# sdroh1027/DiffusionVID

Measured on AMD Instinct MI355X. Metric: frames/sec (1000x600) DiffusionVID-R101 x1, higher is better.
Workload: dtype f16

## Files before the change

diffusionvid_amd/_lib.py:

```python
import ctypes as C
import os

_HERE = os.path.dirname(os.path.abspath(__file__))
LIB_PATH = os.environ.get("DVID_LIB") or os.path.join(_HERE, "libdvid_hip.so")

c_void_p, c_int, c_float, c_int64 = C.c_void_p, C.c_int, C.c_float, C.c_int64
c_float_p = C.POINTER(C.c_float)


class DvidConfig(C.Structure):
    _fields_ = [
        ("hidden_dim", c_int), ("nheads", c_int), ("dim_feedforward", c_int), ("dim_dynamic", c_int),
        ("num_classes", c_int), ("num_cls", c_int), ("num_reg", c_int), ("num_heads", c_int),
        ("num_heads_cond", c_int), ("pooler_resolution", c_int), ("sampling_ratio", c_int),
        ("res_blocks", c_int * 4), ("pixel_mean", c_float * 3), ("pixel_std", c_float * 3),
        ("backbone_type", c_int), ("swin_embed_dim", c_int), ("swin_depths", c_int * 4), ("swin_heads", c_int * 4),
        ("swin_window", c_int),
    ]


SIGNATURES = {
    "dvid_last_error": (C.c_char_p, []),
    "dvid_version": (c_int, []),
    "dvid_model_create": (c_int, [C.POINTER(DvidConfig), C.POINTER(c_void_p)]),
    "dvid_model_destroy": (c_int, [c_void_p]),
    "dvid_model_set_tensor": (c_int, [c_void_p, C.c_char_p, c_void_p, C.POINTER(c_int64), c_int]),
    "dvid_model_finalize": (c_int, [c_void_p]),
    "dvid_model_set_precision": (c_int, [c_void_p, c_int]),
    "dvid_model_take_range_flag": (c_int, [c_void_p, C.POINTER(c_int), c_void_p]),
    "dvid_set_chains": (c_int, [c_void_p, c_int]),
    "dvid_set_stem_layout": (c_int, [c_void_p, c_int]),
    "dvid_workspace_reserve": (c_int, [c_void_p, c_int, c_int, c_int, c_int]),
    "dvid_workspace_generation": (C.c_ulonglong, [c_void_p]),
    "dvid_backbone_resnet_fpn": (c_int, [c_void_p, c_void_p, c_int, c_int, c_int, c_void_p, c_void_p, c_void_p, c_void_p]),
    "dvid_backbone_swin_fpn": (c_int, [c_void_p, c_void_p, c_int, c_int, c_int, c_void_p, c_void_p, c_void_p, c_void_p]),
    "dvid_backbone_resnet_fpn_frames": (c_int, [c_void_p, c_void_p, c_int, c_int, c_int, c_void_p, c_void_p, c_void_p, c_void_p]),
    "dvid_backbone_swin_fpn_frames": (c_int, [c_void_p, c_void_p, c_int, c_int, c_int, c_void_p, c_void_p, c_void_p, c_void_p]),
    "dvid_rcnn_head": (c_int, [c_void_p, c_int, c_int, c_void_p, c_void_p, c_void_p, c_int, c_int, c_int, c_int, c_void_p,
                               c_void_p, C.POINTER(c_int64), c_void_p, c_void_p, c_void_p, c_void_p, c_void_p, c_void_p]),
    "dvid_global_xattn": (c_int, [c_void_p, c_void_p, c_int, c_void_p, c_int, c_void_p, c_void_p]),
    "dvid_global_memory_project": (c_int, [c_void_p, c_void_p, c_int, c_void_p]),
    "dvid_local_memory_project": (c_int, [c_void_p, c_int, c_void_p, c_int, c_int, c_void_p]),
    "dvid_local_xattn": (c_int, [c_void_p, c_int, c_void_p, c_int, c_int, c_int, c_void_p, c_void_p]),
    "dvid_roialign_v2_multilevel": (c_int, [c_void_p, c_void_p, c_void_p, c_int, c_int, c_int, c_int, c_void_p, c_int,
                                            c_void_p, c_void_p, c_void_p]),
    "dvid_roialign_v2_multilevel_f32": (c_int, [c_void_p, c_void_p, c_void_p, c_int, c_int, c_int, c_int, c_void_p, c_int,
                                                c_void_p, c_void_p, c_void_p]),
    "dvid_conv2d_nhwc_f32": (c_int, [c_void_p] * 8 + [c_int] * 12 + [c_void_p]),
    "dvid_mha_f32": (c_int, [c_void_p] * 4 + [c_int] * 7 + [c_int64] * 3 + [c_void_p]),
    "dvid_swin_window_attn_f32": (c_int, [c_void_p] * 4 + [c_int] * 6 + [c_void_p]),
    "dvid_swin_window_attn_f32_ws": (c_int, [c_void_p] * 4 + [c_int] * 7 + [c_void_p]),
    "dvid_dynconv_f32": (c_int, [c_void_p] * 7 + [c_int, c_void_p]),
    "dvid_select_topk_features": (c_int, [c_void_p, c_int, c_int, c_int, c_int, c_int, c_void_p, c_int, c_void_p, c_void_p,
                                          c_void_p]),
    "dvid_counter_normal": (c_int, [c_void_p, C.c_int64, c_int, C.c_uint64, c_void_p]),
    "dvid_noise_to_boxes": (c_int, [c_void_p, c_void_p, c_int, c_float, c_float, c_float, c_void_p]),
    "dvid_ddim_renew_step": (c_int, [c_void_p] * 6 + [c_int] * 3 + [c_float] * 9 + [c_void_p]),
    "dvid_postproc_topk_nms": (c_int, [c_void_p, c_void_p, c_int, c_int, c_int, c_int, c_float, c_float, c_float, c_int,
                                       c_void_p, c_void_p, c_void_p, c_void_p, c_void_p, c_void_p]),
    "dvid_postproc_scratch_bytes": (c_int64, [c_int, c_int, c_int]),
    "dvid_topk_candidates_stream": (c_int, [c_void_p, c_void_p, c_int, c_int, c_int, c_int, c_void_p, c_void_p, c_void_p, c_void_p]),
    "dvid_nms_frames_tiled": (c_int, [c_void_p] * 3 + [c_int, c_int, c_float, c_float, c_float, c_int, c_int] + [c_void_p] * 6),
    "dvid_nms_tiled_scratch_bytes": (c_int64, [c_int, c_int]),
    "dvid_seq_nms_video": (c_int, [c_void_p] * 4 + [c_int] * 3 + [c_void_p] * 4 + [c_int64, c_void_p]),
    "dvid_seq_nms_scratch_bytes": (c_int64, [c_void_p, c_void_p, c_int, c_int]),
    "dvid_cdist": (c_int, [c_void_p, c_int, c_int, c_void_p, c_void_p]),
    "dvid_fps_greedy": (c_int, [c_void_p, c_int, c_int, c_int, c_void_p, c_void_p]),
    "dvid_gather_rows": (c_int, [c_void_p, c_void_p, c_void_p, c_int, c_int, c_void_p]),
    "dvid_conv2d_nhwc_f16": (c_int, [c_void_p, c_void_p, c_void_p, c_void_p, c_void_p] + [c_int] * 13 + [c_void_p]),
    "dvid_bottleneck64_tail_f16": (c_int, [c_void_p] * 10 + [c_int] + [c_void_p] * 2 + [c_int] * 3 + [c_void_p]),
    "dvid_bottleneck128_tail_f16": (c_int, [c_void_p] * 10 + [c_int] * 3 + [c_void_p]),
    "dvid_mha_f16": (c_int, [c_void_p] * 5 + [c_int] * 7 + [c_int64] * 3 + [c_void_p]),
    "dvid_dynconv": (c_int, [c_void_p] * 7 + [c_int, c_void_p]),
    "dvid_add_layernorm": (c_int, [c_void_p] * 5 + [c_int, c_int, c_int, c_void_p]),
    "dvid_swin_pack_relbias": (c_int, [c_void_p, c_int, c_void_p]),
    "dvid_swin_window_attn_f16": (c_int, [c_void_p] * 4 + [c_int] * 6 + [c_void_p]),
    "dvid_swin_pack_relbias_ws": (c_int, [c_void_p, c_int, c_int, c_void_p]),
    "dvid_swin_window_attn_f16_ws": (c_int, [c_void_p] * 4 + [c_int] * 7 + [c_void_p]),
    "dvid_patch_merge_ln": (c_int, [c_void_p] * 5 + [c_int] * 4 + [c_void_p]),
    "dvid_nhwc_from_nchw": (c_int, [c_void_p, c_void_p, c_int, c_int, c_int, c_int, c_void_p]),
    "dvid_nchw_from_nhwc": (c_int, [c_void_p, c_void_p, c_int, c_int, c_int, c_int, c_void_p]),
    "dvid_f32_to_f16": (c_int, [c_void_p, c_void_p, c_int64, c_void_p]),
    "dvid_resize_u8_to_f32": (c_int, [c_void_p, c_int, c_int, c_void_p, c_void_p, c_int, c_int, c_int, c_int, c_void_p, c_void_p, c_int,
                                      c_void_p, c_void_p, c_int, c_void_p]),
    "dvid_igemm_num_configs": (c_int, []),
    "dvid_igemm_set_config": (c_int, [c_int]),
    "dvid_igemm_set_tuning": (c_int, [c_int]),
    "dvid_igemm_tuning_passes": (C.c_longlong, []),
    "dvid_igemm_set_conv3x3": (c_int, [c_int]),
    "dvid_igemm_set_wstat": (c_int, [c_int]),
    "dvid_igemm_set_bottleneck_fusion": (c_int, [c_int]),
    "dvid_set_stem_pool": (c_int, [c_int]),
    "dvid_set_option": (c_int, [C.c_char_p, c_int]),
    "dvid_get_option": (c_int, [C.c_char_p, C.POINTER(c_int)]),
    "dvid_reset_options": (c_int, []),
    "dvid_effective_config": (c_int, [C.c_char_p, c_int]),
    "dvid_profile_enable": (c_int, [c_int]),
    "dvid_profile_reset": (c_int, []),
# ... 54 lines not shown
```

diffusionvid_amd/csrc/dynconv.hip:

```cpp
#include "common.h"
#include "f32_split.h"
#include "igemm_epilogue.h"
#include "kernels.h"
#include "options.h"
#include "roi_taps.h"

namespace {

constexpr int NP = 49;
constexpr int D = 256;
constexpr int DD = 64;
constexpr int A_PITCH = D + 8;
constexpr int H_PITCH = DD + 8;

__device__ __forceinline__ float groups4_sum(float v) {
    v += __shfl_xor(v, 16, 64);
    v += __shfl_xor(v, 32, 64);
    return v;
}

template <bool FUSED_ROI>
__global__ __launch_bounds__(256, 3) void dynconv_kernel(const half_t* __restrict__ roi, const half_t* __restrict__ params,
                                                       const float* __restrict__ g1, const float* __restrict__ b1,
                                                       const float* __restrict__ g2, const float* __restrict__ b2,
                                                       half_t* __restrict__ out, RoiLevels lv, const float* __restrict__ boxes,
                                                       int boxes_per_img, int nbox) {
    extern __shared__ __attribute__((aligned(16))) char smem[];
    half_t* As = reinterpret_cast<half_t*>(smem);
    half_t* Hs = As + 64 * A_PITCH;
    float* red = reinterpret_cast<float*>(Hs + 64 * H_PITCH);

    const int box = FUSED_ROI ? igemm_xcd_remap((int)blockIdx.x, nbox) : (int)blockIdx.x;
    const int tid = threadIdx.x, lane = tid & 63, wave = tid >> 6;
    const int l15 = lane & 15, l4 = lane >> 4;
    const half_t* p1t = params + (long)box * (2 * D * DD);
    const half_t* p2t = p1t + D * DD;
    const half8 zero8 = {0, 0, 0, 0, 0, 0, 0, 0};
    half8 bf[8];
    half8 b2f[4][2];

    if (FUSED_ROI) {
#pragma unroll
        for (int ks = 0; ks < 8; ++ks)
            bf[ks] = *reinterpret_cast<const half8*>(p1t + (wave * 16 + l15) * D + ks * 32 + l4 * 8);
#pragma unroll
        for (int nt = 0; nt < 4; ++nt)
#pragma unroll
            for (int ks = 0; ks < 2; ++ks)
                b2f[nt][ks] = *reinterpret_cast<const half8*>(p2t + (wave * 64 + nt * 16 + l15) * DD + ks * 32 + l4 * 8);
        float macc[8];
        roi_taps::gather_box(lv, boxes, boxes_per_img, box, tid >> 5, tid & 31, macc,
                             [&](int p, half8 o) { *reinterpret_cast<half8*>(As + p * A_PITCH + (tid & 31) * 8) = o; });
        for (int i = tid; i < (64 - NP) * 32; i += 256) *reinterpret_cast<half8*>(As + (NP + (i >> 5)) * A_PITCH + (i & 31) * 8) = zero8;
    } else {
        const half_t* roi_b = roi + (long)box * NP * D;
        for (int i = tid; i < 64 * 32; i += 256) {
            const int r = i >> 5, cv = i & 31;
            const half8 v = *reinterpret_cast<const half8*>(roi_b + (long)(r < NP ? r : 0) * D + cv * 8);
            *reinterpret_cast<half8*>(As + r * A_PITCH + cv * 8) = (r < NP) ? v : zero8;
        }
#pragma unroll
        for (int ks = 0; ks < 8; ++ks)
            bf[ks] = *reinterpret_cast<const half8*>(p1t + (wave * 16 + l15) * D + ks * 32 + l4 * 8);
    }
    __syncthreads();

    float4v acc1[4];
#pragma unroll
    for (int mt = 0; mt < 4; ++mt) acc1[mt] = (float4v){0.f, 0.f, 0.f, 0.f};
#pragma unroll
    for (int ks = 0; ks < 8; ++ks) {
#pragma unroll
        for (int mt = 0; mt < 4; ++mt) {
            const half8 af = *reinterpret_cast<const half8*>(As + (mt * 16 + l15) * A_PITCH + ks * 32 + l4 * 8);
            acc1[mt] = __builtin_amdgcn_mfma_f32_16x16x32_f16(bf[ks], af, acc1[mt], 0, 0, 0);
        }
    }
    if (!FUSED_ROI) {
#pragma unroll
        for (int nt = 0; nt < 4; ++nt)
#pragma unroll
            for (int ks = 0; ks < 2; ++ks)
                b2f[nt][ks] = *reinterpret_cast<const half8*>(p2t + (wave * 64 + nt * 16 + l15) * DD + ks * 32 + l4 * 8);
    }

    float mean[4], rstd[4];
#pragma unroll
    for (int mt = 0; mt < 4; ++mt) {
        const float s = groups4_sum((acc1[mt][0] + acc1[mt][1]) + (acc1[mt][2] + acc1[mt][3]));
        if (l4 == 0) red[(mt * 16 + l15) * 4 + wave] = s;
    }
    __syncthreads();
#pragma unroll
    for (int mt = 0; mt < 4; ++mt) {
        const float4v t = *reinterpret_cast<const float4v*>(red + (mt * 16 + l15) * 4);
        mean[mt] = (t[0] + t[1] + t[2] + t[3]) * (1.f / DD);
    }
    __syncthreads();
#pragma unroll
    for (int mt = 0; mt < 4; ++mt) {
        float s = 0.f;
#pragma unroll
        for (int r = 0; r < 4; ++r) {
            const float c = acc1[mt][r] - mean[mt];
// ... 418 lines not shown
```

diffusionvid_amd/csrc/kernels.h:

```cpp
#pragma once
#include "common.h"

struct IgemmParams {
    const half_t* in;
    const half_t* w;
    const float* bias;
    const void* res;
    void* out;
    int H, W, Cin, Ho, Wo, Cout, KH, KW, stride, pad;
    int M, Kpad, ntaps, ldc, alg_k;
    int relu, out_f32, res_mode, res_f32;
    int splitk;
    long split_stride;
    int tiles_m, tiles_n;
};
int dvid_igemm_launch(const IgemmParams& p, hipStream_t s);
int dvid_igemm2_launch(const IgemmParams& p, hipStream_t s);

bool dvid_conv3x3_halo_supported(const IgemmParams& p);
bool dvid_conv3x3_halo_preferred(const IgemmParams& p);
int dvid_conv3x3_halo_launch(const IgemmParams& p, hipStream_t s);
bool dvid_stem_pool_supported(const IgemmParams& p);
int dvid_stem_pool_launch(const IgemmParams& p, hipStream_t s);

bool dvid_wstat_supported(const IgemmParams& p);
bool dvid_wstat_preferred(const IgemmParams& p);
int dvid_wstat_launch(const IgemmParams& p, hipStream_t s);

bool dvid_bneck64_tail_preferred(int H, int W);
int dvid_bneck128_tail_launch(const half_t* t1, const half_t* w2, const float* b2, const half_t* w3, const float* b3, const half_t* res,
                              const half_t* w1n, const float* b1n, half_t* out, half_t* t1n, int n, int H, int W, hipStream_t s);
int dvid_bneck64_tail_launch(const half_t* t1, const half_t* w2, const float* b2, const half_t* w3, const float* b3, const half_t* res,
                             const half_t* ws, const float* bs, const half_t* w1n, const float* b1n, int n_next, half_t* out, half_t* t1n,
                             int n, int H, int W, hipStream_t s);

struct FrameTable {
    static constexpr int kMax = 32;
    const float* p[kMax];
};
int dvid_prep_images_launch(const float* const* frames, half_t* nhwc8, int n, int h, int w, const float* mean, const float* inv_std,
                            hipStream_t s);
int dvid_prep_images_s2d_launch(const float* const* frames, half_t* s2d16, int n, int h, int w, const float* mean, const float* inv_std,
                                hipStream_t s);
int dvid_maxpool3x3s2_launch(const half_t* in, half_t* out, int n, int h, int w, int c, hipStream_t s);
int dvid_nchw_from_nhwc_launch(const half_t* in, float* out, int n, int h, int w, int c, hipStream_t s);
int dvid_nhwc_from_nchw_launch(const float* in, half_t* out, int n, int h, int w, int c, hipStream_t s);
int dvid_add_layernorm_launch(const float* x, const float* r, const float* g, const float* b, float* y32, half_t* y16,
                              int rows, int d, int relu, hipStream_t s, int nsplit = 1, long split_stride = 0,
                              const float* xbias = nullptr);
int dvid_f32_to_f16_launch(const float* x, half_t* y, long n, hipStream_t s);
int dvid_resize_u8_launch(const unsigned char* src, int h, int w, unsigned char* tmp, float* out, int oh, int ow, int ph, int pw,
                          const int* xbounds, const int* xk, int xksize, const int* ybounds, const int* yk, int yksize, hipStream_t s);
int dvid_modulate_launch(const float* x, const float* scale, int scale_ld, const float* shift, int shift_per_row, int shift_ld,
                         half_t* y16, int rows, int rows_per_frame, int d, hipStream_t s);
int dvid_silu_f16_launch(const float* x, half_t* y, long n, hipStream_t s);

template <typename T>
struct RoiLevelsT {
    const T* feat[3];
    int h[3], w[3];
    float scale[3];
};
using RoiLevels = RoiLevelsT<half_t>;
using RoiLevels32 = RoiLevelsT<float>;
int dvid_roialign_launch(const RoiLevels& lv, int channels, const float* boxes, int n_img, int boxes_per_img, half_t* roi_out,
                         float* mean_out, hipStream_t s);

int dvid_mha_mfma_launch(const half_t* q, const half_t* k, const half_t* v, half_t* out, half_t* vt_scratch, int batch, int lq,
                         int lk, int nheads, int q_ld, int kv_ld, int out_ld, long q_bs, long kv_bs, long out_bs, hipStream_t s);

struct OutProjLnParams {
    const void* x;
    int mode;
    const half_t* wf_hi;
    const half_t* wf_lo;
    const float* w32;
    const float* wscale;
    const float* bias;
    const float* gamma;
    const float* beta;
    float* out;
    int rows, d;
    int* range_flag;
};
int dvid_outproj_ln_launch(const OutProjLnParams& p, hipStream_t s);

constexpr int SWIN_RELBIAS_PITCH = 64;
int dvid_swin_window_attn_launch(const half_t* qkv, const half_t* qkv_bias16, const float* relbias, half_t* out, int batch, int H,
                                 int W, int C, int nheads, int shift, hipStream_t s);
constexpr int SWIN12_RELBIAS_PITCH = 160;
int dvid_swin_window12_attn_launch(const half_t* qkv, const half_t* qkv_bias16, const float* relbias, half_t* out, int batch, int H,
                                   int W, int C, int nheads, int shift, hipStream_t s);
int dvid_patch_merge_ln_launch(const float* x, const float* g, const float* b, half_t* y16, int B, int H, int W, int C, hipStream_t s,
                               float* y32 = nullptr);

int dvid_dynconv_launch(const half_t* roi, const half_t* params, const float* g1, const float* b1, const float* g2,
                        const float* b2, half_t* out, int rows, hipStream_t s);
int dvid_dynconv_roi_launch(const RoiLevels& lv, int channels, const float* boxes, int n_img, int boxes_per_img, const half_t* params,
                            const float* g1, const float* b1, const float* g2, const float* b2, half_t* out, hipStream_t s);

struct HeadTailParams {
    const half_t* x16;
    const float* obj32;
    const half_t* w1f;
    const float* b1;
    const half_t* w2f;
    const float* b2;
    const float* n3g;
    const float* n3b;
    const float* scale;
    int ss_stride, rows_per_frame;
    const float* cond32;
    const half_t* wcf;
    const float* bc;
    int num_cls, num_reg, num_classes, dff;
    const half_t* clsf[4];
    const float* clsg[4];
    const float* clsb[4];
    const half_t* regf[4];
// ... 87 lines not shown
```

diffusionvid_amd/csrc/ops_abi.hip:

```cpp
#include "runtime.h"

extern "C" {
int dvid_roialign_v2_multilevel(const void* p3, const void* p4, const void* p5, int n_frames, int height, int width, int channels,
                                const float* boxes, int boxes_per_frame, void* roi_out, float* mean_out, void* stream) {
    g_err[0] = 0;
    if (height % 32 || width % 32) FAIL(DVID_ERR_ARG, "height/width must be multiples of 32");
    TRY(dvid_roialign_launch(roi_levels<half_t>(p3, p4, p5, height, width, 0, channels), channels, boxes, n_frames, boxes_per_frame, reinterpret_cast<half_t*>(roi_out), mean_out,
                             reinterpret_cast<hipStream_t>(stream)));
    return DVID_OK;
}

int dvid_roialign_v2_multilevel_f32(const float* p3, const float* p4, const float* p5, int n_frames, int height, int width, int channels,
                                    const float* boxes, int boxes_per_frame, float* roi_out, float* mean_out, void* stream) {
    g_err[0] = 0;
    if (height % 32 || width % 32) FAIL(DVID_ERR_ARG, "height/width must be multiples of 32");
    TRY(dvid_f32_roialign_launch(roi_levels<float>(p3, p4, p5, height, width, 0, channels), channels, boxes, n_frames, boxes_per_frame, roi_out, mean_out, reinterpret_cast<hipStream_t>(stream)));
    return DVID_OK;
}

int dvid_conv2d_nhwc_f32(const float* in, const float* w, const void* w_hi, const void* w_lo, const float* bias, const float* row_scale, const float* residual,
                         float* out, int n, int h, int wd, int cin, int cout, int kh, int kw, int stride, int pad, int kpad, int relu, int residual_mode,
                         void* stream) {
    g_err[0] = 0;
    if (cin % 4 || kpad % 16 || kpad < kh * kw * cin || pad < 0) FAIL(DVID_ERR_ARG, "fp32 conv: cin %% 4 == 0, kpad %% 16 == 0, kpad >= kh*kw*cin, pad >= 0");
    ConvW cw;
    cw.w32 = const_cast<float*>(w);
    cw.w16hi = reinterpret_cast<half_t*>(const_cast<void*>(w_hi));
    cw.w16lo = reinterpret_cast<half_t*>(const_cast<void*>(w_lo));
    cw.bias = const_cast<float*>(bias);
    cw.wscale32 = const_cast<float*>(row_scale);
    cw.cin32 = cin;
    cw.cin_real = cin;
    cw.cout = cout;
    cw.kh = kh;
    cw.kw = kw;
    cw.stride = stride;
    cw.pad = pad;
    cw.kpad32 = kpad;
    TRY(conv_run32(cw, in, n, h, wd, out, reinterpret_cast<hipStream_t>(stream), {.relu = relu, .res = residual, .res_mode = residual_mode}));
    return DVID_OK;
}

int dvid_mha_f32(const float* q, const float* k, const float* v, float* out, int batch, int lq, int lk, int nheads, int q_ld, int kv_ld, int out_ld,
                 int64_t q_bs, int64_t kv_bs, int64_t out_bs, void* stream) {
    g_err[0] = 0;
    TRY(dvid_f32_mha_launch(q, k, v, out, batch, lq, lk, nheads, q_ld, kv_ld, out_ld, (long)q_bs, (long)kv_bs, (long)out_bs,
                            reinterpret_cast<hipStream_t>(stream)));
    return DVID_OK;
}

int dvid_swin_window_attn_f32(const float* qkv, const float* qkv_bias, const float* relbias, float* out, int batch, int H, int W, int C,
                              int nheads, int shift, void* stream) {
    g_err[0] = 0;
    if (!qkv || !qkv_bias || !relbias || !out) FAIL(DVID_ERR_ARG, "swin window attention: null pointer");
    if (batch <= 0 || H <= 0 || W <= 0 || nheads <= 0 || shift < 0 || shift >= 7)
        FAIL(DVID_ERR_ARG, "swin window attention: bad sizes (batch %d, %d x %d tokens, %d heads, shift %d)", batch, H, W, nheads, shift);
    const int rc = dvid_f32_swin_window_attn_launch(qkv, qkv_bias, relbias, out, batch, H, W, C, nheads, shift, reinterpret_cast<hipStream_t>(stream));
    if (rc != DVID_OK) FAIL(rc, "swin window attention (fp32): C %d with %d heads on %d x %d x %d tokens is not supported", C, nheads, batch, H, W);
    return DVID_OK;
}

// ... 291 lines not shown
```

diffusionvid_amd/csrc/roi_taps.h:

```cpp
#pragma once

#include "common.h"
#include "kernels.h"

namespace roi_taps {

constexpr int P = 7;
constexpr int G = 2;
constexpr int CV = 32;

typedef unsigned int uint4v __attribute__((ext_vector_type(4)));
__device__ __forceinline__ float mix_fma_lo(unsigned int h2, float w, float acc) {
    float d;
    asm("v_fma_mix_f32 %0, %1, %2, %3 op_sel_hi:[1,0,0]" : "=v"(d) : "v"(h2), "v"(w), "v"(acc));
    return d;
}
__device__ __forceinline__ float mix_fma_hi(unsigned int h2, float w, float acc) {
    float d;
    asm("v_fma_mix_f32 %0, %1, %2, %3 op_sel:[1,0,0] op_sel_hi:[1,0,0]" : "=v"(d) : "v"(h2), "v"(w), "v"(acc));
    return d;
}
__device__ __forceinline__ void tap_fma8(float (&acc)[8], half8 v, float w) {
    const uint4v u = __builtin_bit_cast(uint4v, v);
#pragma unroll
    for (int q = 0; q < 4; ++q) {
        acc[2 * q] = mix_fma_lo(u[q], w, acc[2 * q]);
        acc[2 * q + 1] = mix_fma_hi(u[q], w, acc[2 * q + 1]);
    }
}

struct Tap {
    int lo, hi;
    float wl, wh;
    bool ok;
};

__device__ __forceinline__ Tap axis_tap(float y, int limit) {
    Tap t;
    t.ok = !(y < -1.0f || y > (float)limit);
    if (y <= 0.f) y = 0.f;
    int lo = (int)y;
    int hi;
    if (lo >= limit - 1) {
        hi = lo = limit - 1;
        y = (float)lo;
    } else {
        hi = lo + 1;
    }
    const float l = y - (float)lo;
    t.lo = lo;
    t.hi = hi;
    t.wl = 1.f - l;
    t.wh = l;
    return t;
}

__device__ __forceinline__ int box_level(float bx1, float by1, float bx2, float by2, bool& valid) {
    const float area = (bx2 - bx1) * (by2 - by1);
    valid = area >= 0.f;
    float lvf = floorf(4.f + log2f(sqrtf(area) / 224.f + 1e-8f));
    lvf = fminf(fmaxf(lvf, 3.f), 5.f);
    return valid ? (int)lvf - 3 : 0;
}

template <typename Sink>
__device__ __forceinline__ void gather_box(const RoiLevels& lv, const float* __restrict__ boxes, int boxes_per_img, int box, int grp, int ln,
                                           float (&macc)[8], Sink&& sink) {
    const int img = box / boxes_per_img;
    const float bx1 = boxes[box * 4 + 0], by1 = boxes[box * 4 + 1], bx2 = boxes[box * 4 + 2], by2 = boxes[box * 4 + 3];
    bool valid_box;
    const int level = box_level(bx1, by1, bx2, by2, valid_box);

    const half_t* feat = lv.feat[level];
    const int H = lv.h[level], W = lv.w[level];
    const float sc = lv.scale[level];
    feat += (long)img * H * W * (CV * 8);

    const float x1 = bx1 * sc - 0.5f, y1 = by1 * sc - 0.5f;
    const float x2 = bx2 * sc - 0.5f, y2 = by2 * sc - 0.5f;
    const float bin_w = (x2 - x1) / P, bin_h = (y2 - y1) / P;

#pragma unroll
    for (int e = 0; e < 8; ++e) macc[e] = 0.f;

    for (int p = grp; p < P * P; p += 8) {
        const int ph = p / P, pw = p - ph * P;
        float acc[8];
#pragma unroll
        for (int e = 0; e < 8; ++e) acc[e] = 0.f;
        if (valid_box) {
#pragma unroll
            for (int iy = 0; iy < G; ++iy) {
                const float y = y1 + ph * bin_h + (iy + 0.5f) * bin_h / G;
                const Tap ty = axis_tap(y, H);
#pragma unroll
                for (int ix = 0; ix < G; ++ix) {
                    const float x = x1 + pw * bin_w + (ix + 0.5f) * bin_w / G;
                    const Tap tx = axis_tap(x, W);
                    if (!(ty.ok && tx.ok)) continue;
                    const half8 v1 = *reinterpret_cast<const half8*>(feat + ((long)ty.lo * W + tx.lo) * (CV * 8) + ln * 8);
                    const half8 v2 = *reinterpret_cast<const half8*>(feat + ((long)ty.lo * W + tx.hi) * (CV * 8) + ln * 8);
                    const half8 v3 = *reinterpret_cast<const half8*>(feat + ((long)ty.hi * W + tx.lo) * (CV * 8) + ln * 8);
                    const half8 v4 = *reinterpret_cast<const half8*>(feat + ((long)ty.hi * W + tx.hi) * (CV * 8) + ln * 8);
                    const float w1 = ty.wl * tx.wl, w2 = ty.wl * tx.wh, w3 = ty.wh * tx.wl, w4 = ty.wh * tx.wh;
                    tap_fma8(acc, v1, w1);
                    tap_fma8(acc, v2, w2);
                    tap_fma8(acc, v3, w3);
                    tap_fma8(acc, v4, w4);
                }
            }
        }
        half8 o;
#pragma unroll
        for (int e = 0; e < 8; ++e) {
            acc[e] *= 1.f / (G * G);
            macc[e] += acc[e];
            o[e] = (half_t)acc[e];
        }
        sink(p, o);
    }
}

}
```

diffusionvid_amd/csrc/roialign.hip:

```cpp
#include <stdlib.h>

#include "common.h"
#include "igemm_epilogue.h"
#include "kernels.h"
#include "roi_taps.h"

namespace {

using namespace roi_taps;

__global__ __launch_bounds__(256) void roialign_kernel(RoiLevels lv, const float* __restrict__ boxes, int boxes_per_img,
                                                        half_t* __restrict__ roi_out, float* __restrict__ mean_out, int nbox,
                                                        int xcd_major) {
    __shared__ float red[8][256];
    const int box = xcd_major ? igemm_xcd_remap((int)blockIdx.x, nbox) : (int)blockIdx.x;
    const int tid = threadIdx.x;
    const int grp = tid >> 5, ln = tid & 31;
    float macc[8];
    gather_box(lv, boxes, boxes_per_img, box, grp, ln, macc,
               [&](int p, half8 o) { *reinterpret_cast<half8*>(roi_out + ((long)box * (P * P) + p) * (CV * 8) + ln * 8) = o; });
    if (mean_out) {
#pragma unroll
        for (int e = 0; e < 8; ++e) red[grp][ln * 8 + e] = macc[e];
        __syncthreads();
        float s = 0.f;
#pragma unroll
        for (int g = 0; g < 8; ++g) s += red[g][tid];
        mean_out[(long)box * 256 + tid] = s / (P * P);
    }
}

__global__ __launch_bounds__(256) void f32_roialign_kernel(RoiLevels32 lv, const float* __restrict__ boxes, int boxes_per_img,
                                                            float* __restrict__ roi_out, float* __restrict__ mean_out, int nbox) {
#pragma clang fp contract(off)
    __shared__ float red[8][256];
    const int box = igemm_xcd_remap((int)blockIdx.x, nbox);
    const int img = box / boxes_per_img;
    const int tid = threadIdx.x;
    const int grp = tid >> 5, ln = tid & 31;
    const float bx1 = boxes[box * 4 + 0], by1 = boxes[box * 4 + 1], bx2 = boxes[box * 4 + 2], by2 = boxes[box * 4 + 3];
    bool valid_box;
    const int level = box_level(bx1, by1, bx2, by2, valid_box);
    const int H = lv.h[level], W = lv.w[level];
    const float sc = lv.scale[level];
    const float* feat = lv.feat[level] + (long)img * H * W * 256;
    const float x1 = bx1 * sc - 0.5f, y1 = by1 * sc - 0.5f;
    const float x2 = bx2 * sc - 0.5f, y2 = by2 * sc - 0.5f;
    const float bin_w = (x2 - x1) / P, bin_h = (y2 - y1) / P;
    float macc[8];
#pragma unroll
    for (int e = 0; e < 8; ++e) macc[e] = 0.f;
    for (int pb = grp; pb < P * P; pb += 8) {
        const int ph = pb / P, pw = pb - ph * P;
        float acc[8];
#pragma unroll
        for (int e = 0; e < 8; ++e) acc[e] = 0.f;
        if (valid_box) {
#pragma unroll
            for (int iy = 0; iy < G; ++iy) {
                const float y = y1 + ph * bin_h + (iy + 0.5f) * bin_h / G;
                const Tap ty = axis_tap(y, H);
#pragma unroll
                for (int ix = 0; ix < G; ++ix) {
                    const float x = x1 + pw * bin_w + (ix + 0.5f) * bin_w / G;
                    const Tap tx = axis_tap(x, W);
                    if (!(ty.ok && tx.ok)) continue;
                    const float w4[4] = {ty.wl * tx.wl, ty.wl * tx.wh, ty.wh * tx.wl, ty.wh * tx.wh};
                    const long o4[4] = {(long)ty.lo * W + tx.lo, (long)ty.lo * W + tx.hi, (long)ty.hi * W + tx.lo, (long)ty.hi * W + tx.hi};
#pragma unroll
                    for (int q = 0; q < 4; ++q) {
                        const float4v a = *reinterpret_cast<const float4v*>(feat + o4[q] * 256 + ln * 8);
                        const float4v b = *reinterpret_cast<const float4v*>(feat + o4[q] * 256 + ln * 8 + 4);
#pragma unroll
                        for (int e = 0; e < 4; ++e) {
                            acc[e] += w4[q] * a[e];
                            acc[4 + e] += w4[q] * b[e];
                        }
                    }
                }
            }
        }
#pragma unroll
        for (int e = 0; e < 8; ++e) {
            acc[e] *= 1.f / (G * G);
            macc[e] += acc[e];
        }
        float* o = roi_out + ((long)box * (P * P) + pb) * 256 + ln * 8;
        *reinterpret_cast<float4v*>(o) = (float4v){acc[0], acc[1], acc[2], acc[3]};
        *reinterpret_cast<float4v*>(o + 4) = (float4v){acc[4], acc[5], acc[6], acc[7]};
    }
    if (mean_out) {
#pragma unroll
        for (int e = 0; e < 8; ++e) red[grp][ln * 8 + e] = macc[e];
        __syncthreads();
        float s = 0.f;
#pragma unroll
        for (int g = 0; g < 8; ++g) s += red[g][tid];
        mean_out[(long)box * 256 + tid] = s / (P * P);
    }
}

}

int dvid_roialign_launch(const RoiLevels& lv, int channels, const float* boxes, int n_img, int boxes_per_img, half_t* roi_out,
                         float* mean_out, hipStream_t s) {
    if (channels != 256) return DVID_ERR_UNSUPPORTED;
    const int nbox = n_img * boxes_per_img;
    if (nbox == 0) return DVID_OK;
    hipLaunchKernelGGL(roialign_kernel, dim3(nbox), dim3(256), 0, s, lv, boxes, boxes_per_img, roi_out, mean_out, nbox, 1);
    LAUNCH_CHECK();
    return DVID_OK;
}

int dvid_f32_roialign_launch(const RoiLevels32& lv, int channels, const float* boxes, int n_img, int boxes_per_img, float* roi_out,
                             float* mean_out, hipStream_t s) {
    if (channels != 256) return DVID_ERR_UNSUPPORTED;
    const int nbox = n_img * boxes_per_img;
    if (nbox == 0) return DVID_OK;
    hipLaunchKernelGGL(f32_roialign_kernel, dim3(nbox), dim3(256), 0, s, lv, boxes, boxes_per_img, roi_out, mean_out, nbox);
    LAUNCH_CHECK();
    return DVID_OK;
}
```

diffusionvid_amd/ops.py:

```python
import ctypes as C

import torch

from . import _lib
from ._lib import call, ptr, stream_ptr


def _cuda(t, dtype=None):
    if not t.is_cuda:
        raise _lib.DvidError("libdvid_hip ops need tensors on the GPU (no CPU fallback)")
    if dtype is not None and t.dtype != dtype:
        raise TypeError(f"expected {dtype}, got {t.dtype}")
    return t.contiguous()


def nhwc_from_nchw(x):
    x = _cuda(x, torch.float32)
    n, c, h, w = x.shape
    out = torch.empty((n, h, w, c), dtype=torch.float16, device=x.device)
    call("dvid_nhwc_from_nchw", ptr(x), ptr(out), n, h, w, c, stream_ptr())
    return out


def nchw_from_nhwc(x):
# ... 80 lines not shown
    p3, p4, p5 = (_cuda(f, torch.float32) for f in feats_nhwc)
    boxes = _cuda(boxes, torch.float32)
    n, M = boxes.shape[:2]
    c = p3.shape[-1]
    roi = torch.empty((n * M, 49, c), dtype=torch.float32, device=boxes.device)
    mean = torch.empty((n * M, c), dtype=torch.float32, device=boxes.device) if want_mean else None
    call("dvid_roialign_v2_multilevel_f32", ptr(p3), ptr(p4), ptr(p5), n, height, width, c, ptr(boxes), M, ptr(roi), ptr(mean), stream_ptr())
    return (roi, mean) if want_mean else roi


def mha_f32(q, k, v, nheads):
    q, k, v = _cuda(q, torch.float32), _cuda(k, torch.float32), _cuda(v, torch.float32)
    B, lq, d = q.shape
    lk = k.shape[1]
    out = torch.empty_like(q)
    call("dvid_mha_f32", ptr(q), ptr(k), ptr(v), ptr(out), B, lq, lk, nheads, d, d, d, lq * d, lk * d, lq * d, stream_ptr())
    return out


def dynconv_f32(roi, params, g1, b1, g2, b2):
    roi, params = _cuda(roi, torch.float32), _cuda(params, torch.float32)
    out = torch.empty_like(roi)
    call("dvid_dynconv_f32", ptr(roi), ptr(params), ptr(g1), ptr(b1), ptr(g2), ptr(b2), ptr(out), roi.shape[0], stream_ptr())
    return out


def bottleneck64_tail(t1, w2, b2, w3, b3, residual, w_sc=None, b_sc=None, w1n=None, b1n=None):
    t1 = _cuda(t1, torch.float16)
    n, h, wd, _ = t1.shape
    nn = int(w1n.shape[0]) if w1n is not None else 0
    out = torch.empty((n, h, wd, 256), dtype=torch.float16, device=t1.device)
    t1n = torch.empty((n, h, wd, nn), dtype=torch.float16, device=t1.device) if w1n is not None else None
    call("dvid_bottleneck64_tail_f16", ptr(t1), ptr(w2), ptr(b2), ptr(w3), ptr(b3), ptr(residual), ptr(w_sc), ptr(b_sc), ptr(w1n),
         ptr(b1n), nn, ptr(out), ptr(t1n), n, h, wd, stream_ptr())
    return out, t1n


def bottleneck128_tail(t1, w2, b2, w3, b3, residual, w1n=None, b1n=None):
    t1 = _cuda(t1, torch.float16)
    n, h, wd, _ = t1.shape
    out = torch.empty((n, h, wd, 512), dtype=torch.float16, device=t1.device)
    t1n = torch.empty((n, h, wd, 128), dtype=torch.float16, device=t1.device) if w1n is not None else None
    call("dvid_bottleneck128_tail_f16", ptr(t1), ptr(w2), ptr(b2), ptr(w3), ptr(b3), ptr(residual), ptr(w1n), ptr(b1n), ptr(out),
         ptr(t1n), n, h, wd, stream_ptr())
    return out, t1n


def linear(x16, w_packed, kpad, bias, relu=False, out_f32=True):
    rows, k = x16.shape
    y = conv2d_nhwc(x16.view(rows, 1, 1, k), w_packed, kpad, bias, w_packed.shape[0], 1, 1, 1, 0, relu=relu, out_f32=out_f32)
    return y.view(rows, -1)


def roialign(feats_nhwc, boxes, height, width, want_mean=False):
    p3, p4, p5 = (_cuda(f, torch.float16) for f in feats_nhwc)
    boxes = _cuda(boxes, torch.float32)
    n, M = boxes.shape[:2]
    c = p3.shape[-1]
    roi = torch.empty((n * M, 49, c), dtype=torch.float16, device=boxes.device)
    mean = torch.empty((n * M, c), dtype=torch.float32, device=boxes.device) if want_mean else None
    call("dvid_roialign_v2_multilevel", ptr(p3), ptr(p4), ptr(p5), n, height, width, c, ptr(boxes), M, ptr(roi), ptr(mean),
         stream_ptr())
    return (roi, mean) if want_mean else roi


def mha_f16(q, k, v, nheads):
    def h(t):
        t = _cuda(t)
        if t.dtype == torch.float16:
            return t
        o = torch.empty(t.shape, dtype=torch.float16, device=t.device)
        call("dvid_f32_to_f16", ptr(t), ptr(o), t.numel(), stream_ptr())
        return o
    q, k, v = h(q), h(k), h(v)
    B, lq, d = q.shape
    lk = k.shape[1]
    out = torch.empty_like(q)
    vt = torch.empty((B * nheads * 32 * ((lk + 31) // 32 * 32 + 32),), dtype=torch.float16, device=q.device)
    call("dvid_mha_f16", ptr(q), ptr(k), ptr(v), ptr(out), ptr(vt), B, lq, lk, nheads, d, d, d, lq * d, lk * d, lq * d,
         stream_ptr())
    return out


def dynconv(roi16, params16, g1, b1, g2, b2):
    roi16, params16 = _cuda(roi16, torch.float16), _cuda(params16, torch.float16)
    out = torch.empty_like(roi16)
    call("dvid_dynconv", ptr(roi16), ptr(params16), ptr(g1), ptr(b1), ptr(g2), ptr(b2), ptr(out), roi16.shape[0], stream_ptr())
    return out


def add_layernorm(x, r, g, b, relu=False):
    x = _cuda(x, torch.float32)
    y = torch.empty_like(x)
    call("dvid_add_layernorm", ptr(x), ptr(r), ptr(g), ptr(b), ptr(y), x.shape[0], x.shape[1], int(relu), stream_ptr())
    return y


def _swin_relbias_pitch(window):
    return (window * window + 31) // 32 * 32


def swin_pack_relbias(table, window=7):
    table = table.detach().cpu().contiguous()
    if table.dtype != torch.float32 or table.dim() != 2 or table.shape[0] != (2 * window - 1) ** 2:
        raise TypeError(f"expected a float32 [{(2 * window - 1) ** 2}, heads] table, got {table.dtype} {tuple(table.shape)}")
    out = torch.empty((table.shape[1], window * window, _swin_relbias_pitch(window)), dtype=torch.float32)
    if window == 7:
        call("dvid_swin_pack_relbias", ptr(table), table.shape[1], ptr(out))
    else:
        call("dvid_swin_pack_relbias_ws", ptr(table), table.shape[1], window, ptr(out))
    return out


def _swin_window_attn(name, dtype, qkv, qkv_bias, relbias, B, H, W, nheads, shift, out, window):
    qkv, qkv_bias, relbias = _cuda(qkv, dtype), _cuda(qkv_bias, dtype), _cuda(relbias, torch.float32)
# ... 419 lines not shown
```

include/dvid_hip.h:

```cpp
#ifndef DVID_HIP_H
#define DVID_HIP_H

#include <stdint.h>

#ifdef __cplusplus
extern "C" {
#endif

#define DVID_OK 0
#define DVID_ERR_ARG 1
#define DVID_ERR_HIP 2
#define DVID_ERR_UNSUPPORTED 3
#define DVID_ERR_STATE 4

#define DVID_MAX_CLASSES 1280

typedef struct dvid_model dvid_model;

typedef struct dvid_config {
    int hidden_dim;
    int nheads;
    int dim_feedforward;
    int dim_dynamic;
    int num_classes;
// ... 3 lines not shown
    int num_heads_cond;
    int pooler_resolution;
    int sampling_ratio;
    int res_blocks[4];
    float pixel_mean[3];
    float pixel_std[3];
    int backbone_type;
    int swin_embed_dim;
    int swin_depths[4];
    int swin_heads[4];
    int swin_window;
} dvid_config;

const char* dvid_last_error(void);
int dvid_version(void);

int dvid_model_create(const dvid_config* cfg, dvid_model** out);
int dvid_model_destroy(dvid_model* m);
int dvid_model_set_tensor(dvid_model* m, const char* name, const float* data, const int64_t* shape, int ndim);
int dvid_model_set_precision(dvid_model* m, int precision);
int dvid_model_take_range_flag(dvid_model* m, int* exceeded, void* stream);
int dvid_model_finalize(dvid_model* m);
int dvid_workspace_reserve(dvid_model* m, int max_frames, int height, int width, int boxes_per_frame);
unsigned long long dvid_workspace_generation(const dvid_model* m);

int dvid_set_chains(dvid_model* m, int nchain);

int dvid_set_stem_layout(dvid_model* m, int space_to_depth);

int dvid_backbone_resnet_fpn(dvid_model* m, const float* images, int n, int height, int width, void* p3, void* p4, void* p5,
                             void* stream);
int dvid_backbone_resnet_fpn_frames(dvid_model* m, const float* const* frames, int n, int height, int width, void* p3, void* p4, void* p5,
                                    void* stream);

int dvid_backbone_swin_fpn(dvid_model* m, const float* images, int n, int height, int width, void* p3, void* p4, void* p5,
                           void* stream);
int dvid_backbone_swin_fpn_frames(dvid_model* m, const float* const* frames, int n, int height, int width, void* p3, void* p4, void* p5,
                                  void* stream);

int dvid_rcnn_head(dvid_model* m, int head_index, int is_cond, const void* p3, const void* p4, const void* p5, int n_frames,
                   int height, int width, int boxes_per_frame, const float* boxes, const float* pro_features,
                   const int64_t* t, const float* cond, float* logits, float* boxes_out, float* obj_features,
                   int* bad_box_flag, void* stream);

int dvid_global_xattn(dvid_model* m, const float* query, int rows, const float* memory, int lk, float* out, void* stream);
int dvid_global_memory_project(dvid_model* m, const float* memory, int lk, void* stream);

int dvid_local_memory_project(dvid_model* m, int stage, const float* memory, int lk, int groups, void* stream);
int dvid_local_xattn(dvid_model* m, int stage, const float* query, int rows, int groups, int lk, float* out, void* stream);

int dvid_roialign_v2_multilevel(const void* p3, const void* p4, const void* p5, int n_frames, int height, int width,
                                int channels, const float* boxes, int boxes_per_frame, void* roi_out ,
                                float* mean_out , void* stream);
int dvid_roialign_v2_multilevel_f32(const float* p3, const float* p4, const float* p5, int n_frames, int height, int width, int channels,
                                    const float* boxes, int boxes_per_frame, float* roi_out, float* mean_out, void* stream);
int dvid_conv2d_nhwc_f32(const float* in, const float* w, const void* w_hi, const void* w_lo, const float* bias, const float* row_scale, const float* residual,
                         float* out, int n, int h, int wd, int cin, int cout, int kh, int kw, int stride, int pad, int kpad, int relu, int residual_mode,
                         void* stream);
int dvid_mha_f32(const float* q, const float* k, const float* v, float* out, int batch, int lq, int lk, int nheads, int q_ld, int kv_ld, int out_ld,
                 int64_t q_bs, int64_t kv_bs, int64_t out_bs, void* stream);
int dvid_swin_window_attn_f32(const float* qkv, const float* qkv_bias, const float* relbias, float* out, int batch, int H, int W, int C,
                              int nheads, int shift, void* stream);
int dvid_swin_window_attn_f32_ws(const float* qkv, const float* qkv_bias, const float* relbias, float* out, int batch, int H, int W, int C,
                                 int nheads, int shift, int window, void* stream);
int dvid_dynconv_f32(const float* roi, const float* params, const float* g1, const float* b1, const float* g2, const float* b2, float* out,
                     int rows, void* stream);
int dvid_select_topk_features(const float* logits, int n_frames, int m, int num_classes, int k1, int k2, const float* feats,
                              int hidden, float* out_k1, float* out_k2, void* stream);
int dvid_counter_normal(float* out, int64_t per_image, int n_images, uint64_t key0, void* stream);
int dvid_noise_to_boxes(const float* x, float* boxes, int n, float snr_scale, float img_w, float img_h, void* stream);
int dvid_ddim_renew_step(const float* logits, const float* boxes, const float* x_t, const float* noise, const float* fresh,
                         float* x_next, int n_frames, int m, int c, float img_w, float img_h, float snr_scale,
                         float sqrt_recip_ac, float sqrt_recipm1_ac, float sqrt_ac_next, float coef_c, float sigma, float keep_thr,
                         void* stream);
#define DVID_NMS_MAX_CANDIDATES 4096
int dvid_postproc_topk_nms(const float* logits, const float* boxes, int nsets, int n_frames, int m, int c, float img_w,
                           float img_h, float iou_threshold, int use_nms, float* out_boxes, float* out_scores,
                           int* out_labels, int* out_counts, void* scratch, void* stream);
int64_t dvid_postproc_scratch_bytes(int nsets, int n_frames, int m);
int dvid_topk_candidates_stream(const float* logits, const float* boxes, int nsets, int n_frames, int m, int c, float* cand_boxes,
                                float* cand_scores, int* cand_labels, void* stream);
int dvid_nms_frames_tiled(const float* cand_boxes, const float* cand_scores, const int* cand_labels, int n_frames, int n, float img_w,
                          float img_h, float iou_threshold, int use_nms, int out_cap, float* out_boxes, float* out_scores,
                          int* out_labels, int* out_counts, void* scratch, void* stream);
int64_t dvid_nms_tiled_scratch_bytes(int n_frames, int n);
#define DVID_SEQ_NMS_MAX_SCRATCH_BYTES (1ll << 30)
#define DVID_SEQ_NMS_ERR_ROUNDS (1 << 30)
#define DVID_SEQ_NMS_ERR_COUNTS (1 << 29)
int dvid_seq_nms_video(const float* dets, const int* counts, const int* class_counts, const int* video_starts, int n_videos, int cap,
                       int num_classes, unsigned char* keep, float* scores, int* status, void* scratch, int64_t scratch_bytes, void* stream);
int64_t dvid_seq_nms_scratch_bytes(const int* class_counts, const int* video_starts, int n_videos, int num_classes);
int dvid_cdist(const float* x, int n, int d, float* dist, void* stream);
int dvid_fps_greedy(const float* dist, int n, int m, int bs_emul, int* idx, void* stream);
int dvid_gather_rows(const float* x, const int* idx, float* y, int m, int d, void* stream);
int dvid_conv2d_nhwc_f16(const void* in, const void* w, const float* bias, const void* residual, void* out, int n, int h,
                         int wd, int cin, int cout, int kh, int kw, int stride, int pad, int kpad, int relu, int out_f32,
                         int residual_mode, void* stream);
int dvid_bottleneck64_tail_f16(const void* t1, const void* w2, const float* b2, const void* w3, const float* b3, const void* residual,
                               const void* w_shortcut, const float* b_shortcut, const void* w1_next, const float* b1_next, int next_channels,
                               void* out, void* t1_next, int n, int h, int wd, void* stream);
int dvid_bottleneck128_tail_f16(const void* t1, const void* w2, const float* b2, const void* w3, const float* b3, const void* residual,
                                const void* w1_next, const float* b1_next, void* out, void* t1_next, int n, int h, int wd, void* stream);
int dvid_mha_f16(const void* q, const void* k, const void* v, void* out, void* vt_scratch, int batch, int lq, int lk, int nheads,
                 int q_ld, int kv_ld, int out_ld, int64_t q_bs, int64_t kv_bs, int64_t out_bs, void* stream);
int dvid_dynconv(const void* roi, const void* params, const float* g1, const float* b1, const float* g2, const float* b2,
                 void* out, int rows, void* stream);
// ... 43 lines not shown
```

Before: 2302.

## Precompute RoIAlign axis taps in shared memory and issue bin loads branch-free

Replaces the default RoIAlign gather with a version where 28 threads compute per-axis bilinear tap offsets and weights once per box into shared memory. Each lane group then issues all 16 half8 loads for a bin at once, with invalid taps redirected to a zero line instead of branching, and a scheduling barrier keeps the loads ahead of the accumulation. The old walk is kept as a serial variant, which the dynconv fused path now calls explicitly. This costs a __syncthreads and shared storage per block and drops per-sample coordinate recomputation and divergent branches.

```diff
diff --git a/diffusionvid_amd/_lib.py b/diffusionvid_amd/_lib.py
--- a/diffusionvid_amd/_lib.py
+++ b/diffusionvid_amd/_lib.py
@@ -44,6 +44,8 @@
     "dvid_local_xattn": (c_int, [c_void_p, c_int, c_void_p, c_int, c_int, c_int, c_void_p, c_void_p]),
     "dvid_roialign_v2_multilevel": (c_int, [c_void_p, c_void_p, c_void_p, c_int, c_int, c_int, c_int, c_void_p, c_int,
                                             c_void_p, c_void_p, c_void_p]),
+    "dvid_roialign_v2_multilevel_serial": (c_int, [c_void_p, c_void_p, c_void_p, c_int, c_int, c_int, c_int, c_void_p, c_int,
+                                                   c_void_p, c_void_p, c_void_p]),
     "dvid_roialign_v2_multilevel_f32": (c_int, [c_void_p, c_void_p, c_void_p, c_int, c_int, c_int, c_int, c_void_p, c_int,
                                                 c_void_p, c_void_p, c_void_p]),
     "dvid_conv2d_nhwc_f32": (c_int, [c_void_p] * 8 + [c_int] * 12 + [c_void_p]),
diff --git a/diffusionvid_amd/csrc/dynconv.hip b/diffusionvid_amd/csrc/dynconv.hip
--- a/diffusionvid_amd/csrc/dynconv.hip
+++ b/diffusionvid_amd/csrc/dynconv.hip
@@ -49,7 +49,7 @@
             for (int ks = 0; ks < 2; ++ks)
                 b2f[nt][ks] = *reinterpret_cast<const half8*>(p2t + (wave * 64 + nt * 16 + l15) * DD + ks * 32 + l4 * 8);
         float macc[8];
-        roi_taps::gather_box(lv, boxes, boxes_per_img, box, tid >> 5, tid & 31, macc,
+        roi_taps::gather_box_serial(lv, boxes, boxes_per_img, box, tid >> 5, tid & 31, macc,
                              [&](int p, half8 o) { *reinterpret_cast<half8*>(As + p * A_PITCH + (tid & 31) * 8) = o; });
         for (int i = tid; i < (64 - NP) * 32; i += 256) *reinterpret_cast<half8*>(As + (NP + (i >> 5)) * A_PITCH + (i & 31) * 8) = zero8;
     } else {
diff --git a/diffusionvid_amd/csrc/kernels.h b/diffusionvid_amd/csrc/kernels.h
--- a/diffusionvid_amd/csrc/kernels.h
+++ b/diffusionvid_amd/csrc/kernels.h
@@ -65,6 +65,8 @@
 using RoiLevels32 = RoiLevelsT<float>;
 int dvid_roialign_launch(const RoiLevels& lv, int channels, const float* boxes, int n_img, int boxes_per_img, half_t* roi_out,
                          float* mean_out, hipStream_t s);
+int dvid_roialign_serial_launch(const RoiLevels& lv, int channels, const float* boxes, int n_img, int boxes_per_img, half_t* roi_out,
+                                float* mean_out, hipStream_t s);
 
 int dvid_mha_mfma_launch(const half_t* q, const half_t* k, const half_t* v, half_t* out, half_t* vt_scratch, int batch, int lq,
                          int lk, int nheads, int q_ld, int kv_ld, int out_ld, long q_bs, long kv_bs, long out_bs, hipStream_t s);
diff --git a/diffusionvid_amd/csrc/ops_abi.hip b/diffusionvid_amd/csrc/ops_abi.hip
--- a/diffusionvid_amd/csrc/ops_abi.hip
+++ b/diffusionvid_amd/csrc/ops_abi.hip
@@ -7,6 +7,15 @@
     if (height % 32 || width % 32) FAIL(DVID_ERR_ARG, "height/width must be multiples of 32");
     TRY(dvid_roialign_launch(roi_levels<half_t>(p3, p4, p5, height, width, 0, channels), channels, boxes, n_frames, boxes_per_frame, reinterpret_cast<half_t*>(roi_out), mean_out,
                              reinterpret_cast<hipStream_t>(stream)));
+    return DVID_OK;
+}
+
+int dvid_roialign_v2_multilevel_serial(const void* p3, const void* p4, const void* p5, int n_frames, int height, int width, int channels,
+                                       const float* boxes, int boxes_per_frame, void* roi_out, float* mean_out, void* stream) {
+    g_err[0] = 0;
+    if (height % 32 || width % 32) FAIL(DVID_ERR_ARG, "height/width must be multiples of 32");
+    TRY(dvid_roialign_serial_launch(roi_levels<half_t>(p3, p4, p5, height, width, 0, channels), channels, boxes, n_frames, boxes_per_frame,
+                                    reinterpret_cast<half_t*>(roi_out), mean_out, reinterpret_cast<hipStream_t>(stream)));
     return DVID_OK;
 }
 
diff --git a/diffusionvid_amd/csrc/roi_taps.h b/diffusionvid_amd/csrc/roi_taps.h
--- a/diffusionvid_amd/csrc/roi_taps.h
+++ b/diffusionvid_amd/csrc/roi_taps.h
@@ -64,7 +64,7 @@
 }
 
 template <typename Sink>
-__device__ __forceinline__ void gather_box(const RoiLevels& lv, const float* __restrict__ boxes, int boxes_per_img, int box, int grp, int ln,
+__device__ __forceinline__ void gather_box_serial(const RoiLevels& lv, const float* __restrict__ boxes, int boxes_per_img, int box, int grp, int ln,
                                            float (&macc)[8], Sink&& sink) {
     const int img = box / boxes_per_img;
     const float bx1 = boxes[box * 4 + 0], by1 = boxes[box * 4 + 1], bx2 = boxes[box * 4 + 2], by2 = boxes[box * 4 + 3];
@@ -121,4 +121,105 @@
     }
 }
 
-}
+struct __attribute__((aligned(16))) TapRec {
+    int lo, hi;
+    float wl, wh;
+};
+struct BoxTaps {
+    TapRec t[2][P * G];
+};
+
+static __device__ __attribute__((aligned(512))) unsigned int g_zero_line[128];
+
+__device__ __forceinline__ float sample_coord(float c1, int pb, int s, float bin) {
+#pragma clang fp contract(off)
+    const float t = ((float)s + 0.5f) * bin;
+    return fmaf(bin, (float)pb, c1) + t * 0.5f;
+}
+
+template <typename Sink>
+__device__ __forceinline__ void gather_box(const RoiLevels& lv, const float* __restrict__ boxes, int boxes_per_img, int box, int grp, int ln,
+                                           float (&macc)[8], Sink&& sink) {
+    static_assert(G == 2 && P == 7, "7 x 7 bins of 2 x 2 samples over 8 lane groups: seven rounds, the last one for bin 48 alone");
+    __shared__ BoxTaps T;
+    const int img = box / boxes_per_img;
+    const float bx1 = boxes[box * 4 + 0], by1 = boxes[box * 4 + 1], bx2 = boxes[box * 4 + 2], by2 = boxes[box * 4 + 3];
+    bool valid_box;
+    const int level = box_level(bx1, by1, bx2, by2, valid_box);
+    const half8 zero8 = {0, 0, 0, 0, 0, 0, 0, 0};
+#pragma unroll
+    for (int e = 0; e < 8; ++e) macc[e] = 0.f;
+    if (!valid_box) {
+        for (int p = grp; p < P * P; p += 8) sink(p, zero8);
+        return;
+    }
+
+    const int H = lv.h[level], W = lv.w[level];
+    const float sc = lv.scale[level];
+    const char* feat = reinterpret_cast<const char*>(lv.feat[level] + (long)img * H * W * (CV * 8)) + ln * 16;
+    const char* zero = reinterpret_cast<const char*>(g_zero_line) + ln * 16;
+
+    const int tid = grp * 32 + ln;
+    if (tid < 2 * P * G) {
+        const int ax = tid >= P * G, i = tid - ax * (P * G);
+        const float c1 = fmaf(ax ? bx1 : by1, sc, -0.5f), c2 = fmaf(ax ? bx2 : by2, sc, -0.5f);
+        const float bin = (c2 - c1) / P;
+        const Tap t = axis_tap(sample_coord(c1, i >> 1, i & 1, bin), ax ? W : H);
+        const int pitch = ax ? CV * 16 : W * (CV * 16);
+        T.t[ax][i] = TapRec{t.ok ? t.lo * pitch : -1, t.ok ? t.hi * pitch : -1, t.wl, t.wh};
+    }
+    __syncthreads();
+
+    half8 v[G * G][4];
+    float w[G * G][4];
+    auto request = [&](int p) {
+        const bool bin_ok = p < P * P;
+        const int ph = bin_ok ? p / P : 0, pw = bin_ok ? p - ph * P : 0;
+#pragma unroll
+        for (int iy = 0; iy < G; ++iy) {
+            const TapRec ty = T.t[0][ph * G + iy];
+#pragma unroll
+            for (int ix = 0; ix < G; ++ix) {
+                const TapRec tx = T.t[1][pw * G + ix];
+                const bool ok = bin_ok & ((ty.lo | tx.lo) >= 0);
+                const char* base = ok ? feat : zero;
+                const unsigned m = ok ? ~0u : 0u;
+                const int s = iy * G + ix;
+                v[s][0] = *reinterpret_cast<const half8*>(base + ((unsigned)(ty.lo + tx.lo) & m));
+                v[s][1] = *reinterpret_cast<const half8*>(base + ((unsigned)(ty.lo + tx.hi) & m));
+                v[s][2] = *reinterpret_cast<const half8*>(base + ((unsigned)(ty.hi + tx.lo) & m));
+                v[s][3] = *reinterpret_cast<const half8*>(base + ((unsigned)(ty.hi + tx.hi) & m));
+                w[s][0] = ty.wl * tx.wl;
+                w[s][1] = ty.wl * tx.wh;
+                w[s][2] = ty.wh * tx.wl;
+                w[s][3] = ty.wh * tx.wh;
+            }
+        }
+    };
+    auto finish = [&](int p) {
+        float acc[8];
+#pragma unroll
+        for (int e = 0; e < 8; ++e) acc[e] = 0.f;
+#pragma unroll
+        for (int s = 0; s < G * G; ++s)
+#pragma unroll
+            for (int q = 0; q < 4; ++q) tap_fma8(acc, v[s][q], w[s][q]);
+        half8 o;
+#pragma unroll
+        for (int e = 0; e < 8; ++e) {
+            acc[e] *= 1.f / (G * G);
+            macc[e] += acc[e];
+            o[e] = (half_t)acc[e];
+        }
+        if (p < P * P) sink(p, o);
+    };
+    int p = grp;
+#pragma unroll 1
+    for (int k = 0; k < 7; ++k, p += 8) {
+        request(p);
+        __builtin_amdgcn_sched_barrier(0);
+        finish(p);
+    }
+}
+
+}
diff --git a/diffusionvid_amd/csrc/roialign.hip b/diffusionvid_amd/csrc/roialign.hip
--- a/diffusionvid_amd/csrc/roialign.hip
+++ b/diffusionvid_amd/csrc/roialign.hip
@@ -9,6 +9,7 @@
 
 using namespace roi_taps;
 
+template <bool SERIAL>
 __global__ __launch_bounds__(256) void roialign_kernel(RoiLevels lv, const float* __restrict__ boxes, int boxes_per_img,
                                                         half_t* __restrict__ roi_out, float* __restrict__ mean_out, int nbox,
                                                         int xcd_major) {
@@ -17,8 +18,9 @@
     const int tid = threadIdx.x;
     const int grp = tid >> 5, ln = tid & 31;
     float macc[8];
-    gather_box(lv, boxes, boxes_per_img, box, grp, ln, macc,
-               [&](int p, half8 o) { *reinterpret_cast<half8*>(roi_out + ((long)box * (P * P) + p) * (CV * 8) + ln * 8) = o; });
+    auto sink = [&](int p, half8 o) { *reinterpret_cast<half8*>(roi_out + ((long)box * (P * P) + p) * (CV * 8) + ln * 8) = o; };
+    if (SERIAL) gather_box_serial(lv, boxes, boxes_per_img, box, grp, ln, macc, sink);
+    else gather_box(lv, boxes, boxes_per_img, box, grp, ln, macc, sink);
     if (mean_out) {
 #pragma unroll
         for (int e = 0; e < 8; ++e) red[grp][ln * 8 + e] = macc[e];
@@ -107,7 +109,17 @@
     if (channels != 256) return DVID_ERR_UNSUPPORTED;
     const int nbox = n_img * boxes_per_img;
     if (nbox == 0) return DVID_OK;
-    hipLaunchKernelGGL(roialign_kernel, dim3(nbox), dim3(256), 0, s, lv, boxes, boxes_per_img, roi_out, mean_out, nbox, 1);
+    hipLaunchKernelGGL(roialign_kernel<false>, dim3(nbox), dim3(256), 0, s, lv, boxes, boxes_per_img, roi_out, mean_out, nbox, 1);
+    LAUNCH_CHECK();
+    return DVID_OK;
+}
+
+int dvid_roialign_serial_launch(const RoiLevels& lv, int channels, const float* boxes, int n_img, int boxes_per_img, half_t* roi_out,
+                                float* mean_out, hipStream_t s) {
+    if (channels != 256) return DVID_ERR_UNSUPPORTED;
+    const int nbox = n_img * boxes_per_img;
+    if (nbox == 0) return DVID_OK;
+    hipLaunchKernelGGL(roialign_kernel<true>, dim3(nbox), dim3(256), 0, s, lv, boxes, boxes_per_img, roi_out, mean_out, nbox, 1);
     LAUNCH_CHECK();
     return DVID_OK;
 }
diff --git a/diffusionvid_amd/ops.py b/diffusionvid_amd/ops.py
--- a/diffusionvid_amd/ops.py
+++ b/diffusionvid_amd/ops.py
@@ -156,15 +156,15 @@
     return y.view(rows, -1)
 
 
-def roialign(feats_nhwc, boxes, height, width, want_mean=False):
+def roialign(feats_nhwc, boxes, height, width, want_mean=False, serial_walk=False):
     p3, p4, p5 = (_cuda(f, torch.float16) for f in feats_nhwc)
     boxes = _cuda(boxes, torch.float32)
     n, M = boxes.shape[:2]
     c = p3.shape[-1]
     roi = torch.empty((n * M, 49, c), dtype=torch.float16, device=boxes.device)
     mean = torch.empty((n * M, c), dtype=torch.float32, device=boxes.device) if want_mean else None
-    call("dvid_roialign_v2_multilevel", ptr(p3), ptr(p4), ptr(p5), n, height, width, c, ptr(boxes), M, ptr(roi), ptr(mean),
-         stream_ptr())
+    call("dvid_roialign_v2_multilevel_serial" if serial_walk else "dvid_roialign_v2_multilevel", ptr(p3), ptr(p4), ptr(p5), n, height, width,
+         c, ptr(boxes), M, ptr(roi), ptr(mean), stream_ptr())
     return (roi, mean) if want_mean else roi
 
 
diff --git a/include/dvid_hip.h b/include/dvid_hip.h
--- a/include/dvid_hip.h
+++ b/include/dvid_hip.h
@@ -79,6 +79,8 @@
 int dvid_roialign_v2_multilevel(const void* p3, const void* p4, const void* p5, int n_frames, int height, int width,
                                 int channels, const float* boxes, int boxes_per_frame, void* roi_out ,
                                 float* mean_out , void* stream);
+int dvid_roialign_v2_multilevel_serial(const void* p3, const void* p4, const void* p5, int n_frames, int height, int width,
+                                       int channels, const float* boxes, int boxes_per_frame, void* roi_out, float* mean_out, void* stream);
 int dvid_roialign_v2_multilevel_f32(const float* p3, const float* p4, const float* p5, int n_frames, int height, int width, int channels,
                                     const float* boxes, int boxes_per_frame, float* roi_out, float* mean_out, void* stream);
 int dvid_conv2d_nhwc_f32(const float* in, const float* w, const void* w_hi, const void* w_lo, const float* bias, const float* row_scale, const float* residual,
```

New measurement: 2291. No clear change (-0.5%).
